# bitbank2/JPEGDEC

Hardware: NVIDIA H100
Metric: Mpixels/sec baseline 4:2:0 decode (batch) (higher is better)
Workload: dtype int16/int32 (u8 pixels)

## Files before the change

jpegdec_b200/csrc/jd_core.h:

```cpp
#ifndef JD_CORE_H
#define JD_CORE_H

#include <stdint.h>
#include <string.h>

#ifdef __CUDACC__
#define JD_HD __host__ __device__ __forceinline__
#define JD_HDM __host__ __device__ __forceinline__
#else
#define JD_HD static inline
#define JD_HDM inline
#endif

#define JD_LUT_DC_SIZE 1152
#define JD_LUT_AC_SIZE 2048
#define JD_LUT_ACF_SIZE 2048
#define JD_LUT_DC(t) ((t) * JD_LUT_DC_SIZE)
#define JD_LUT_AC(t) (2 * JD_LUT_DC_SIZE + (t) * JD_LUT_AC_SIZE)
#define JD_LUT_ACF(t) (2 * JD_LUT_DC_SIZE + 2 * JD_LUT_AC_SIZE + (t) * JD_LUT_ACF_SIZE)
#define JD_LUT_ENTRIES (2 * JD_LUT_DC_SIZE + 2 * JD_LUT_AC_SIZE + 2 * JD_LUT_ACF_SIZE)
#define JD_ACF_RARE 0x80u
#define JD_ACF_PACK(len, rs) ((uint32_t)((len) + ((rs) & 15u)) | ((uint32_t)(len) << 8) | (((uint32_t)(rs) & 15u) << 16) | \
                              ((((rs) == 0u) ? 128u : (((uint32_t)(rs) >> 4) + 1u)) << 24) | \
                              (((((rs) & 15u) >= 10u) || ((len) + ((rs) & 15u) >= 18u)) ? JD_ACF_RARE : 0u))

#define JD_REC_PER_BYTE 6u
#define JD_REC_SLOT_SLACK 128u
#define JD_REC_INDEX(byte_off, slot) (((JD_REC_PER_BYTE * (uint32_t)(byte_off)) & ~7u) + JD_REC_SLOT_SLACK * (uint32_t)(slot))
#define JD_REC_CAP(nbytes) (JD_REC_PER_BYTE * (uint32_t)(nbytes) + JD_REC_SLOT_SLACK - 8u)
#define JD_REC_BLOCK_MAX 126u

typedef unsigned long long jd_u64;

JD_HD jd_u64 jd_pack_hdr(uint32_t rec_index, int dc, uint32_t ncoef, uint32_t big, uint32_t hi, uint32_t colmask)
{
    return (jd_u64)rec_index | ((jd_u64)(uint16_t)(int16_t)dc << 32) | ((jd_u64)(ncoef & 63u) << 48) |
           ((jd_u64)(big & 1u) << 54) | ((jd_u64)(hi & 1u) << 55) | ((jd_u64)(colmask & 0xFFu) << 56);
}
#define JD_HDR_REC(h) ((uint32_t)(h))
#define JD_HDR_DC(h) ((int)(short)(uint16_t)((h) >> 32))
#define JD_HDR_NCOEF(h) ((uint32_t)((h) >> 48) & 63u)
#define JD_HDR_BIG(h) ((uint32_t)((h) >> 54) & 1u)
#define JD_HDR_HI(h) ((uint32_t)((h) >> 55) & 1u)
#define JD_HDR_COLMASK(h) ((uint32_t)((h) >> 56) & 0xFFu)

#define JD_TPOS_INIT { \
    0, 8, 1, 2, 9, 16, 24, 17, 10, 3, 4, 11, 18, 25, 32, 40, \
    33, 26, 19, 12, 5, 6, 13, 20, 27, 34, 41, 48, 56, 49, 42, 35, \
    28, 21, 14, 7, 15, 22, 29, 36, 43, 50, 57, 58, 51, 44, 37, 30, \
    23, 31, 38, 45, 52, 59, 60, 53, 46, 39, 47, 54, 61, 62, 55, 63 }
#define JD_TRANSPOSE6(x) ((((x) & 7u) << 3) | ((x) >> 3))

#define JD_DEZIGZAG_INIT { \
    0, 1, 8, 16, 9, 2, 3, 10, 17, 24, 32, 25, 18, 11, 4, 5, \
    12, 19, 26, 33, 40, 48, 41, 34, 27, 20, 13, 6, 7, 14, 21, 28, \
    35, 42, 49, 56, 57, 50, 43, 36, 29, 22, 15, 23, 30, 37, 44, 51, \
    58, 59, 52, 45, 38, 31, 39, 46, 53, 60, 61, 54, 47, 55, 62, 63 }

#define JD_JW_INIT 0x543210u
#define JD_JW_ONES 0x111111u

JD_HD uint32_t jd_jw_ckpt(uint32_t jw)
{
    uint32_t t = (jw + 0x222222u) & 0x888888u;
    uint32_t m = t | (t - (t >> 3));
    return jw & ~m;
}

typedef struct {
    uint32_t blk;
    uint32_t seg;
    uint32_t j1;
    uint16_t field;
    uint8_t s;
    uint8_t p7;
    uint32_t ord;
    uint32_t img;
} JDEvent;

JD_HD void jd_patch_record(uint16_t *rec, jd_u64 hdr, uint32_t ord, int v)
{
    const uint32_t ri = JD_HDR_REC(hdr);
    if (JD_HDR_BIG(hdr)) rec[ri + 2u * ord + 1u] = (uint16_t)(int16_t)v;
    else rec[ri + ord] = (uint16_t)((rec[ri + ord] & 0xFC00u) | ((uint32_t)v & 0x3FFu));
}

JD_HD int jd_event_value(const JDEvent *e, uint32_t jc)
{
    int lost = 8 * (int)jc + e->p7 + e->s - 64;
    uint32_t f = e->field;
    if (lost > 0) {
        if (lost >= e->s) f = 0; else f &= ~((1u << lost) - 1u);
    }
    int v = (int)f;
    if (!(e->field >> (e->s - 1))) v -= (1 << e->s) - 1;
    return v;
}

typedef struct {
    const uint8_t *data;
    uint32_t start;
    uint32_t end;
    uint32_t nmcu;
    uint32_t bpm;
    uint32_t ncomp;
    uint32_t tsel;
    uint32_t rec_index0;
    uint32_t rec_cap;
    uint32_t seg;
    uint32_t blk0;
    uint32_t al;
    uint32_t img;
    uint32_t *ring;
    uint16_t *stage;
    uint32_t skip_bits;
    uint32_t blk_first;
    uint32_t nblk;
    uint32_t midstream;
    int32_t pred[3];
} JDSegIn;
JD_HD void jd_segin_whole_interval(JDSegIn *in)
{
    in->skip_bits = 0; in->blk_first = 0; in->nblk = 0; in->midstream = 0; in->pred[0] = in->pred[1] = in->pred[2] = 0;
}

typedef struct {
    uint32_t jmap;
    int32_t err_mcu;
    uint32_t status;
    uint32_t nrec;
    uint32_t nblk_done;
#ifdef JD_ENTROPY_PROBE
    long long probe[4];
    uint32_t probe_sym;
#endif
} JDSegOut;

#if defined(JD_ENTROPY_PROBE) && defined(__CUDA_ARCH__)
#define JD_PROBE(...) __VA_ARGS__
#else
#define JD_PROBE(...)
#endif

#define JD_SEG_OK 0
#define JD_SEG_BADCODE 1
#define JD_SEG_OVERFLOW 2
#define JD_SEG_BADSIZE 3
#define JD_SEG_MISSING 4

#ifdef __CUDACC__
#define JD_LD8(p) (*(p))
#else
#define JD_LD8(p) (*(p))
#endif

JD_HD uint32_t jd_tposw(uint32_t t) { return t | (((t >> 2) & 1u) << 23) | ((1u << (t >> 3)) << 24); }
#define JD_BF_HI(bf) (((bf) >> 23) & 1u)
#define JD_BF_COLMASK(bf) ((bf) >> 24)
#define JD_BF_MASK 0xFF800000u

#define JD_MODE_BASELINE 0
#define JD_MODE_DC_SCAN 1
#define JD_MODE_PARSE_AC 2
#define JD_MODE_STORE_LOW 3
JD_HD uint32_t jd_bswap32(uint32_t w)
{
#ifdef __CUDA_ARCH__
    return __byte_perm(w, 0, 0x0123);
#else
    return __builtin_bswap32(w);
#endif
}

JD_HD int jd_extend_top(uint32_t x, uint32_t s)
{
    const uint32_t neg = ~(uint32_t)((int)x >> 31);
    const uint32_t y = x ^ neg;
#ifdef __CUDA_ARCH__
    const uint32_t mag = s ? __funnelshift_r(y, 0u, 32u - s) : 0u;
#else
    const uint32_t mag = s ? (y >> (32u - s)) : 0u;
#endif
    return (int)((mag ^ neg) - neg);
}

typedef struct { uint32_t x, y, z, w; } jd_u128;
JD_HD jd_u128 jd_ld128(const uint8_t *p)
{
    jd_u128 r;
#ifdef __CUDA_ARCH__
    const uint4 v = *reinterpret_cast<const uint4 *>(p);
    r.x = v.x; r.y = v.y; r.z = v.z; r.w = v.w;
#else
    memcpy(&r, p, 16);
#endif
    return r;
}

#ifdef __CUDA_ARCH__
struct JDTab16 {
    uint32_t base;
    __device__ __forceinline__ JDTab16(const uint16_t *p) : base((uint32_t)__cvta_generic_to_shared(p)) { asm volatile("" : "+r"(base)); }
    __device__ __forceinline__ uint32_t at(uint32_t i) const { uint16_t v; asm("ld.shared.u16 %0, [%1];" : "=h"(v) : "r"(base + 2u * i)); return v; }
};
struct JDTab32 {
    uint32_t base;
    __device__ __forceinline__ JDTab32(const uint32_t *p) : base((uint32_t)__cvta_generic_to_shared(p)) { asm volatile("" : "+r"(base)); }
    __device__ __forceinline__ uint32_t at(uint32_t i) const { uint32_t v; asm("ld.shared.u32 %0, [%1];" : "=r"(v) : "r"(base + 4u * i)); return v; }
};
#else
struct JDTab16 { const uint16_t *p; JDTab16(const uint16_t *q) : p(q) {} uint32_t at(uint32_t i) const { return p[i]; } };
struct JDTab32 { const uint32_t *p; JDTab32(const uint32_t *q) : p(q) {} uint32_t at(uint32_t i) const { return p[i]; } };
#endif

template <typename EventSink, int MODE = JD_MODE_BASELINE, bool CLEAN = false>
JD_HD void jd_decode_segment(const JDSegIn &in, const uint16_t *lut ,
                             const uint32_t *tposw ,
                             jd_u64 *blk_hdr , uint16_t *rec ,
                             EventSink &sink, JDSegOut &out)
{
    const uint32_t *words = (const uint32_t *)in.data;
    const uint32_t endw = (in.end + 3u) >> 2;
    const uint32_t wlast = in.end >> 2;
    uint32_t wi = in.start >> 2;
    uint32_t wnext = (!CLEAN && wi < endw) ? words[wi] : 0u;
    uint32_t skip = CLEAN ? 0u : (in.start & 3u);
    uint32_t ffp = 0;
    uint32_t eos = 0;
    jd_u64 bb = 0;
    int nb = 0;
    const uint8_t *const cbase = in.data + in.start;
    const uint32_t nchunk = CLEAN ? ((in.end - in.start + 15u) >> 4) : 0u;
    const jd_u128 zero128 = {0u, 0u, 0u, 0u};
    uint32_t *const ring = in.ring;
    uint32_t rd = 0, wr = 0, gi = 0;
    jd_u128 pa = zero128, pb = zero128;
    bool pend = false;
    auto ring_put = [&](uint32_t at, const jd_u128 &v) {
#ifdef __CUDA_ARCH__
        *reinterpret_cast<uint4 *>(ring + at) = make_uint4(v.x, v.y, v.z, v.w);
#else
        ring[at] = v.x; ring[at + 1] = v.y; ring[at + 2] = v.z; ring[at + 3] = v.w;
#endif
    };
    auto chunk = [&](uint32_t i) { return (i < nchunk) ? jd_ld128(cbase + 16u * i) : zero128; };
    auto topup = [&]() {
        if (pend) { ring_put(wr & 31u, pa); ring_put((wr + 4u) & 31u, pb); wr += 8u; }
        pend = (32u - (wr - rd)) >= 8u;
        if (pend) { pa = chunk(gi); pb = chunk(gi + 1u); gi += 2u; }
    };
    if (CLEAN) {
        for (uint32_t i = 0; i < 4u; i++) ring_put(4u * i, chunk(i));
        wr = 16u; gi = 4u;
        topup();
    }
    auto refill = [&]() {
#ifndef JD_REFILL_STRAIGHT
        if (CLEAN) {
            if (nb <= 32) {
                while (rd == wr) topup();
                const uint32_t w = ring[rd & 31u];
                rd++;
                bb |= (jd_u64)jd_bswap32(w) << (32 - nb);
                nb += 32;
            }
        } else
#endif
        if (CLEAN) {
            const bool need = nb <= 32;
            if (need && rd == wr) { do topup(); while (rd == wr); }
            const uint32_t w = jd_bswap32(ring[rd & 31u]);
            const uint32_t sh = need ? (uint32_t)(32 - nb) : 0u;
            const jd_u64 add = (jd_u64)w << sh;
            bb |= need ? add : 0ull;
            rd += need ? 1u : 0u;
            nb += need ? 32 : 0;
        } else
        while (nb <= 32) {
            const uint32_t w = wnext;
            wi++;
            wnext = (wi < endw) ? words[wi] : 0u;
            if ((((((~w) - 0x01010101u) & w & 0x80808080u)) | skip | ffp | eos | (uint32_t)(wi > wlast)) == 0u) {
                bb |= (jd_u64)jd_bswap32(w) << (32 - nb);
                nb += 32;
            } else if (eos) {
                nb = 64;
            } else {
                for (int i = 0; i < 4; i++) {
                    const uint32_t c = (w >> (8 * i)) & 0xFFu;
                    if (skip) { skip--; continue; }
                    if (eos) break;
                    if (wi - 1u == (in.end >> 2) && (uint32_t)i >= (in.end & 3u)) { eos = 1; break; }
                    if (ffp) {
                        ffp = 0;
                        if (c != 0u) { eos = 1; break; }
                        bb |= (jd_u64)0xFFu << (56 - nb);
                        nb += 8;
                        continue;
                    }
                    if (c == 0xFFu) { ffp = 1; continue; }
                    bb |= (jd_u64)c << (56 - nb);
                    nb += 8;
                }
                if (wi >= endw && !eos && nb <= 32) eos = 1;
            }
        }
    };

    int pred0 = in.pred[0], pred1 = in.pred[1], pred2 = in.pred[2];
    uint32_t jw = JD_JW_INIT;
    uint32_t p7 = in.skip_bits & 7u;
    if (CLEAN) {
        for (uint32_t skip = in.skip_bits; skip != 0u;) {
            refill();
            const uint32_t d = skip < 32u ? skip : 32u;
            bb <<= d; nb -= (int)d; skip -= d;
        }
    }
    uint32_t ro = 0;
#ifdef __CUDA_ARCH__
    size_t rec_g = __cvta_generic_to_global(rec);
    asm volatile("" : "+l"(rec_g));
#define JD_REC_ST(i, val) asm volatile("st.global.u16 [%0], %1;" ::"l"(rec_g + 2ull * (i)), "h"((uint16_t)(val)) : "memory")
#else
#define JD_REC_ST(i, val) (rec[(i)] = (uint16_t)(val))
#endif
    uint16_t *const stage = in.stage;
    bool direct = false;
    auto flush_chunk = [&](uint32_t first) {
#ifdef __CUDA_ARCH__
        const uint4 c = *reinterpret_cast<const uint4 *>(stage);
        asm volatile("st.global.v4.u32 [%0], {%1, %2, %3, %4};" ::"l"(rec_g + 2ull * first), "r"(c.x), "r"(c.y), "r"(c.z), "r"(c.w) : "memory");
#else
        memcpy(rec + first, stage, 16);
#endif
    };
    auto put = [&](uint32_t val) {
        if (!direct) {
            stage[ro & 7u] = (uint16_t)val;
            ro++;
            if ((ro & 7u) == 0u) flush_chunk(ro - 8u);
        } else {
            JD_REC_ST(ro, val);
            ro++;
            if ((ro & 7u) == 0u) direct = false;
        }
    };
    auto go_direct = [&]() {
        if (!direct) {
            for (uint32_t i = ro & ~7u; i < ro; i++) JD_REC_ST(i, stage[i & 7u]);
            direct = (ro & 7u) != 0u;
        }
    };
    int err = -1;
    bool last_was_eob = true;
    const JDTab16 T(lut);
    const JDTab32 T32((const uint32_t *)lut);
    const JDTab32 TP(tposw);

    const uint32_t nluma = (in.ncomp == 3) ? in.bpm - 2 : in.bpm;
    const uint32_t nblk_total = in.nblk ? in.nblk : in.nmcu * in.bpm;
    uint32_t sched = 0;
    for (uint32_t i = 0; i < in.bpm && i < 8u; i++) {
        const uint32_t c = (i < nluma) ? 0u : (i - nluma + 1u);
        sched |= (c | (((in.tsel >> (2 * c)) & 1u) << 2) | (((in.tsel >> (2 * c + 1)) & 1u) << 3)) << (4 * i);
    }
    const uint32_t bsh_end = 4u * in.bpm;
    uint32_t bsh = 4u * in.blk_first;
    constexpr uint32_t LIMIT = (MODE == JD_MODE_STORE_LOW) ? 5u : 64u;
    uint32_t b = 0;

    JD_PROBE(long long pt[4] = {0, 0, 0, 0}; long long pc0 = clock64(), pc1; uint32_t nsym = 0;)
#define JD_PROBE_MARK(s) JD_PROBE(pc1 = clock64(); pt[s] += pc1 - pc0; pc0 = pc1;)
    for (; b < nblk_total; b++) {
        const uint32_t cur = (sched >> bsh) & 15u;
        JD_PROBE_MARK(3)
        if (CLEAN) topup();
        JD_PROBE_MARK(0)
        refill();
        jw = jd_jw_ckpt(jw);
        int dcval;
        {
            const uint32_t w16 = (uint32_t)(bb >> 48);
            const uint32_t e = T.at(JD_LUT_DC((cur >> 2) & 1u) + ((w16 >= 0xF800u) ? (1024u + ((w16 >> 4) & 0x7Fu)) : (w16 >> 6)));
            if (e == 0u) { err = JD_SEG_BADCODE; break; }
            const uint32_t len = e >> 8, s = e & 15u;
            bb <<= len;
            const int v = jd_extend_top((uint32_t)(bb >> 32), s);
            bb <<= s;
            nb -= (int)(len + s);
            uint32_t t = p7 + len;
            jw += (t >> 3) * JD_JW_ONES;
            if (s != 0u && len + s > 6u) jw = jd_jw_ckpt(jw);
            t = (t & 7u) + s;
            jw += (t >> 3) * JD_JW_ONES;
            p7 = t & 7u;
            const uint32_t comp = cur & 3u;
            const int pv = ((comp == 0u) ? pred0 : ((comp == 1u) ? pred1 : pred2)) + ((MODE == JD_MODE_DC_SCAN) ? (int)((uint32_t)v << in.al) : v);
            pred0 = (comp == 0u) ? pv : pred0;
            pred1 = (comp == 1u) ? pv : pred1;
            pred2 = (comp >= 2u) ? pv : pred2;
            dcval = pv;
        }
        JD_PROBE_MARK(1)
        const uint32_t r0 = ro;
        uint32_t bflags = 0, bigm = 0;
        if (MODE != JD_MODE_DC_SCAN) {
            if (MODE != JD_MODE_PARSE_AC && in.rec_cap - ro < JD_REC_BLOCK_MAX) { err = JD_SEG_OVERFLOW; break; }
            uint32_t tacf = JD_LUT_ACF(cur >> 3) >> 1;
#if defined(__CUDA_ARCH__) && !defined(JD_NO_LAUNDER)
            asm volatile("" : "+r"(tacf));
#endif
            uint32_t k = 1;
            do {
                JD_PROBE(nsym++;)
                refill();
                jw = jd_jw_ckpt(jw);
                const uint32_t hi = (uint32_t)(bb >> 32);
                uint32_t e = T32.at(tacf + (hi >> 22));
                if (e == 0u) {
                    const uint32_t e16 = (hi >= 0xFC000000u) ? T.at(JD_LUT_AC(cur >> 3) + 1024u + ((hi >> 16) & 0x3FFu)) : 0u;
                    if (e16 == 0u) { err = JD_SEG_BADCODE; break; }
                    e = JD_ACF_PACK(e16 >> 8, e16 & 0xFFu) | JD_ACF_RARE;
                }
                const uint32_t tot = e & 0x1Fu, len = (e >> 8) & 0xFFu, s = (e >> 16) & 0xFFu;
#ifdef __CUDA_ARCH__
                const uint32_t x = __funnelshift_l((uint32_t)bb, hi, len);
                const uint32_t mag = __funnelshift_r(x, 0u, 32u - s);
#else
                const uint32_t x = (uint32_t)((bb << len) >> 32);
                const uint32_t mag = s ? (x >> (32u - s)) : 0u;
#endif
                const int v = (int)(mag - (~(uint32_t)((int)x >> 31) & ~(0xFFFFFFFFu << s)));
                bb <<= tot;
                nb -= (int)tot;
                const uint32_t kn = k + (e >> 24);
                if (MODE != JD_MODE_PARSE_AC && s != 0u && kn <= LIMIT) {
                    const uint32_t tw = TP.at(kn - 1u);
                    bflags |= tw;
                    if (((e | bigm) & JD_ACF_RARE) != 0u) {
                        if (s > 11u) { err = JD_SEG_BADSIZE; break; }
                        if (len + s >= 18u) {
                            const uint32_t t1 = p7 + len;
                            const uint32_t j1 = jw + (t1 >> 3) * JD_JW_ONES;
                            const int q7 = (int)(t1 & 7u);
                            if (((j1 + 0x222222u) & 0x888888u) != 0u) {
                                bool any = false;
                                for (int c = 0; c < 6; c++) {
                                    const int jc = (int)((j1 >> (4 * c)) & 15u);
                                    if (8 * jc + q7 + (int)s > 64) any = true;
                                }
                                if (any) {
                                    JDEvent ev;
                                    ev.blk = in.blk0 + b;
                                    ev.seg = in.seg;
                                    ev.j1 = j1;
                                    ev.field = (uint16_t)(x >> (32u - s));
                                    ev.s = (uint8_t)s;
                                    ev.p7 = (uint8_t)q7;
                                    ev.ord = bigm ? (ro - r0) >> 1 : (ro - r0);
                                    ev.img = in.img;
                                    sink.push(ev);
                                }
                            }
                        }
                        if (s >= 10u && !bigm) {
                            const uint32_t ncoef = ro - r0;
                            go_direct();
                            uint16_t *const rec0 = rec + r0;
                            for (uint32_t i = ncoef; i-- > 0u;) {
                                const uint32_t r = rec0[i];
                                rec0[2u * i] = (uint16_t)(r >> 10);
                                rec0[2u * i + 1u] = (uint16_t)(int16_t)((int)(r << 22) >> 22);
                            }
                            ro += ncoef;
                            direct = true;
                            bigm = JD_ACF_RARE;
                        }
                        if (bigm) {
                            put(tw & 63u);
                            put((uint32_t)v & 0xFFFFu);
                        } else {
                            put((tw << 10) | ((uint32_t)v & 0x3FFu));
                        }
                    } else {
                        put((tw << 10) | ((uint32_t)v & 0x3FFu));
                    }
                }
                {
                    const uint32_t t = p7 + tot;
                    jw += (t >> 3) * JD_JW_ONES;
                    p7 = t & 7u;
                }
                k = kn;
            } while (k < 64u);
            if (err >= 0) break;
            last_was_eob = (k >= 128u);
        }
        JD_PROBE_MARK(2)
        {
            const uint32_t nrec = ro - r0;
            const uint32_t cnt = (bigm ? ((nrec >> 1) << 16) | (1u << 22) : (nrec << 16));
            const uint32_t ridx0 = in.rec_index0 + r0;
            blk_hdr[b] = (jd_u64)ridx0 | ((jd_u64)((bflags & JD_BF_MASK) | cnt | ((uint32_t)dcval & 0xFFFFu)) << 32);
        }
        bsh += 4u;
        if (bsh == bsh_end) bsh = 0u;
    }
    JD_PROBE_MARK(3)
    JD_PROBE(for (int i = 0; i < 4; i++) out.probe[i] = pt[i]; out.probe_sym = nsym;)
#undef JD_PROBE_MARK
    if (!direct && (ro & 7u) != 0u) flush_chunk(ro & ~7u);
    if (err >= 0) {
        out.err_mcu = (int32_t)((b + in.blk_first) / in.bpm);
        for (uint32_t bb2 = b; bb2 < nblk_total; bb2++) blk_hdr[bb2] = jd_pack_hdr(in.rec_index0, 0, 0, 0, 0, 0);
    }
    out.status = (err < 0) ? (uint32_t)JD_SEG_OK : (uint32_t)err;
    if (err < 0) {
        out.err_mcu = -1;
        if (!in.midstream) {
            if (!last_was_eob) jw = jd_jw_ckpt(jw);
            if (p7) jw += JD_JW_ONES;
        }
    }
    out.jmap = jw;
    out.nrec = ro;
    out.nblk_done = b;
#undef JD_REC_ST
}


JD_HD uint32_t jd_range(int v)
{
    int s = (int)((uint32_t)v << 17) >> 22;
    s += 128;
    s = s < 0 ? 0 : s;
    s = s > 255 ? 255 : s;
    return (uint32_t)s;
}

JD_HD int jd_mh2(int x, int K)
{
#ifdef __CUDA_ARCH__
    return (((int)((uint32_t)x << 18) >> 16) * K) >> 16;
#else
    return (int)(((int64_t)(int32_t)((uint32_t)x << 18) * (int64_t)K) >> 32);
#endif
}

#define JD_K0414 (1697 * 4)
#define JD_K1414 (5793 * 4)
#define JD_K1847 (7568 * 4)
#define JD_K2613 (10703 * 2)
#define JD_K1082 (4433 * 4)

JD_HD void jd_col_sse16(const int d[8], bool rows47_empty, int o[8])
{
    int T0, T1, T2, T3, T4, T5, T6, T7;
    if (rows47_empty) {
        const int d0 = d[0], d1 = d[1], d2 = d[2], d3 = d[3];
        int t12 = jd_mh2(d2, JD_K0414);
        T0 = d0 + d2; T3 = d0 - d2; T1 = d0 + t12; T2 = d0 - t12;
        T7 = d1 + d3;
        int t11 = jd_mh2(d1 - d3, JD_K1414);
        int z5 = jd_mh2(d1 - d3, JD_K1847);
        t12 = 2 * jd_mh2(d3, JD_K2613) + z5;
        T6 = t12 - T7;
        T5 = t11 - T6;
        T4 = (jd_mh2(d1, JD_K1082) - z5) + T5;
    } else {
        int t10 = d[0] + d[4], t11 = d[0] - d[4];
        int t13 = d[2] + d[6];
        int t12 = jd_mh2(d[2] - d[6], JD_K1414) - t13;
        T0 = t10 + t13; T3 = t10 - t13; T1 = t11 + t12; T2 = t11 - t12;
        int z13 = d[5] + d[3], z10 = d[5] - d[3];
        int z11 = d[1] + d[7], z12 = d[1] - d[7];
        T7 = z11 + z13;
        t11 = jd_mh2(z11 - z13, JD_K1414);
        int z5 = jd_mh2(z10 + z12, JD_K1847);
        t12 = 2 * jd_mh2(z10, -JD_K2613) + z5;
        T6 = t12 - T7;
        T5 = t11 - T6;
        T4 = (jd_mh2(z12, JD_K1082) - z5) + T5;
    }
    o[0] = T0 + T7; o[1] = T1 + T6; o[2] = T2 + T5; o[3] = T3 - T4;
    o[4] = T3 + T4; o[5] = T2 - T5; o[6] = T1 - T6; o[7] = T0 - T7;
}

JD_HD void jd_col_scalar(const int m[8], const int q[8], bool rows47_empty, int o[8])
{
    int tmp0, tmp1, tmp2, tmp3, tmp4, tmp5, tmp6, tmp7, tmp10, tmp11, tmp12, tmp13, z5, z10, z11, z12, z13;
    if (rows47_empty) {
        tmp10 = m[0] * q[0];
        tmp1 = m[2] * q[2];
        tmp12 = (tmp1 * 106) >> 8;
        tmp0 = tmp10 + tmp1; tmp3 = tmp10 - tmp1; tmp1 = tmp10 + tmp12; tmp2 = tmp10 - tmp12;
        tmp4 = m[1] * q[1];
        if (m[3] != 0) {
            tmp5 = m[3] * q[3];
            tmp7 = tmp4 + tmp5;
            tmp11 = ((tmp4 - tmp5) * 362) >> 8;
            z5 = ((tmp4 - tmp5) * 473) >> 8;
            tmp12 = ((-tmp5 * -669) >> 8) + z5;
            tmp6 = tmp12 - tmp7;
            tmp5 = tmp11 - tmp6;
            tmp10 = ((tmp4 * 277) >> 8) - z5;
            tmp4 = tmp10 + tmp5;
        } else {
            tmp7 = tmp4;
            tmp5 = (145 * tmp4) >> 8;
            tmp6 = (217 * tmp4) >> 8;
            tmp4 = (-51 * tmp4) >> 8;
        }
    } else {
        tmp0 = m[0] * q[0];
        tmp2 = m[4] * q[4];
        tmp10 = tmp0 + tmp2; tmp11 = tmp0 - tmp2;
        tmp1 = m[2] * q[2];
        tmp3 = m[6] * q[6];
        tmp13 = tmp1 + tmp3;
        tmp12 = (((tmp1 - tmp3) * 362) >> 8) - tmp13;
        tmp0 = tmp10 + tmp13; tmp3 = tmp10 - tmp13; tmp1 = tmp11 + tmp12; tmp2 = tmp11 - tmp12;
        tmp5 = m[3] * q[3];
        tmp6 = m[5] * q[5];
        z13 = tmp6 + tmp5; z10 = tmp6 - tmp5;
        tmp4 = m[1] * q[1];
        tmp7 = m[7] * q[7];
        z11 = tmp4 + tmp7; z12 = tmp4 - tmp7;
        tmp7 = z11 + z13;
        tmp11 = ((z11 - z13) * 362) >> 8;
        z5 = ((z10 + z12) * 473) >> 8;
        tmp12 = ((z10 * -669) >> 8) + z5;
        tmp6 = tmp12 - tmp7;
        tmp5 = tmp11 - tmp6;
        tmp10 = ((z12 * 277) >> 8) - z5;
        tmp4 = tmp10 + tmp5;
    }
    o[0] = tmp0 + tmp7; o[1] = tmp1 + tmp6; o[2] = tmp2 + tmp5; o[3] = tmp3 - tmp4;
    o[4] = tmp3 + tmp4; o[5] = tmp2 - tmp5; o[6] = tmp1 - tmp6; o[7] = tmp0 - tmp7;
}

#define JD_MS8(x, K) (((x) * (K)) >> 8)
JD_HD void jd_row_terms(const int p[8], uint32_t colmask, int t[8])
{
    int tmp0, tmp1, tmp2, tmp3, tmp4, tmp5, tmp6, tmp7;
    if ((colmask & 0xf0u) == 0u) {
        if ((colmask & 0xfcu) == 0u) {
            tmp0 = tmp1 = tmp2 = tmp3 = p[0];
            tmp7 = p[1];
            tmp6 = JD_MS8(tmp7, 217);
            tmp5 = JD_MS8(tmp7, 145);
            tmp4 = -JD_MS8(tmp7, 51);
        } else {
            int tmp10 = p[0], tmp13 = p[2];
            int tmp12 = JD_MS8(tmp13, 106);
            tmp0 = tmp10 + tmp13; tmp3 = tmp10 - tmp13; tmp1 = tmp10 + tmp12; tmp2 = tmp10 - tmp12;
            int z13 = p[3], z11 = p[1];
            tmp7 = z11 + z13;
            int tmp11 = JD_MS8(z11 - z13, 362);
            int z5 = JD_MS8(z11 - z13, 473);
            tmp10 = JD_MS8(z11, 277) - z5;
            tmp12 = JD_MS8(z13, 669) + z5;
            tmp6 = tmp12 - tmp7;
            tmp5 = tmp11 - tmp6;
            tmp4 = tmp10 + tmp5;
// ... 233 lines not shown
```

jpegdec_b200/csrc/jd_host.c:

```c
#include <stdio.h>
#include <string.h>
#include <stdlib.h>
#include <math.h>
#include "jd_internal.h"
#include "jd_resize.h"
#include "jd_reduce.h"

#define HUFF_TABLEN 273

static unsigned be16(const uint8_t *p) { return ((unsigned)p[0] << 8) | p[1]; }

static unsigned tiff16(const uint8_t *p, int mot) { return mot ? ((unsigned)p[0] << 8) | p[1] : ((unsigned)p[1] << 8) | p[0]; }
static unsigned tiff32(const uint8_t *p, int mot)
{
    return mot ? ((unsigned)p[0] << 24) | ((unsigned)p[1] << 16) | ((unsigned)p[2] << 8) | p[3]
               : ((unsigned)p[3] << 24) | ((unsigned)p[2] << 16) | ((unsigned)p[1] << 8) | p[0];
}

static int tiff_value(const uint8_t *p, int mot)
{
    int type = (int)tiff16(p + 2, mot);
    if (tiff16(p + 4, mot) > 1) type = 4;
    switch (type) {
        case 3: return (int)tiff16(p + 8, mot);
// ... 167 lines not shown
        off += (int)len;
    }
    if (marker != 0xFFDA) return fail(info, JPEG_DECODE_ERROR);
    off -= (int)len;
    if (off + 3 > size) return fail(info, JPEG_DECODE_ERROR);
    int slen = (int)be16(s + off);
    off += 2;
    int nc = s[off++];
    info->p.ncomp_in_scan = (uint8_t)nc;
    slen -= 3;
    if (nc >= 1 && nc <= 4 && slen == nc * 2 + 3 && off + nc * 2 + 3 <= size) {
        int bad = 0;
        for (int i = 0; i < nc && !bad; i++) {
            unsigned cc = s[off++], c = s[off++];
            int j;
            for (j = 0; j < 4; j++) if (info->p.comp_id[j] == cc) break;
            if (j == 4) { bad = 1; break; }
            if ((c & 0xF) > 3 || (c & 0xF0) > 0x30) { bad = 1; break; }
            info->p.comp_dc[j] = (uint8_t)(c >> 4);
            info->p.comp_ac[j] = (uint8_t)(c & 0xF);
        }
        if (!bad) {
            info->p.scan_start = s[off++];
            info->p.scan_end = s[off++];
            info->approx = s[off++];
        }
    }
    info->scan_offset = off;
    info->p.scan_offset = off;
    if (!(prog_tables && info->mode == 0xC2) && !jd_check_huffman(info)) return fail(info, JPEG_UNSUPPORTED_FEATURE);

    if (info->ncomp != 1 && info->ncomp != 3) return fail(info, JPEG_UNSUPPORTED_FEATURE);
    switch (info->subsample) {
        case 0x00: case 0x11: info->mcu_w = 8; info->mcu_h = 8; info->bpm = (info->ncomp == 3) ? 3 : 1; break;
        case 0x21: info->mcu_w = 16; info->mcu_h = 8; info->bpm = 4; break;
        case 0x12: info->mcu_w = 8; info->mcu_h = 16; info->bpm = 4; break;
        case 0x22: info->mcu_w = 16; info->mcu_h = 16; info->bpm = 6; break;
        default: return fail(info, JPEG_UNSUPPORTED_FEATURE);
    }
    if (info->width <= 0 || info->height <= 0) return fail(info, JPEG_DECODE_ERROR);
    info->mcus_x = (info->width + info->mcu_w - 1) / info->mcu_w;
    info->mcus_y = (info->height + info->mcu_h - 1) / info->mcu_h;
    info->tsel = 0;
    info->tables_ok = 1;
    for (int c = 0; c < info->ncomp; c++) {
        if (info->p.comp_dc[c] > 1 || info->p.comp_ac[c] > 1) info->tables_ok = 0;
        info->tsel |= (info->p.comp_dc[c] & 1) << (2 * c);
        info->tsel |= (info->p.comp_ac[c] & 1) << (2 * c + 1);
    }
    info->error = JPEG_SUCCESS;
    return 1;
}

int jd_check_huffman(const JDInfo *info)
{
    const uint8_t *hv = info->p.huffvals;
    for (int t = 0; t < 4; t++) {
        if (!(info->p.huff_defined & (1u << t))) continue;
        const uint8_t *bits = hv + t * HUFF_TABLEN;
        unsigned cc = 0;
        for (int n = 1; n <= 16; n++) {
            int cnt = bits[n - 1];
            if (n > 12 && cnt > 0) return 0;
            while (cnt--) {
                int is_long = (n >= 5) && ((cc >> (n - 5)) == 0x1F);
                if (!is_long && n > 6) return 0;
                cc++;
            }
            cc <<= 1;
        }
    }
    if (info->mode == 0xC2) return 1;
    for (int t = 0; t < 4; t++) {
        if (!(info->p.huff_defined & (1u << (t + 4)))) continue;
        if (t >= 2) return 0;
        const uint8_t *bits = hv + (t + 4) * HUFF_TABLEN;
        unsigned cc = 0;
        for (int n = 1; n <= 16; n++) {
            int cnt = bits[n - 1];
            while (cnt--) {
                int is_long = (n >= 6) && ((cc >> (n - 6)) == 0x3F);
                if (!is_long && n > 10) return 0;
                cc++;
            }
            cc <<= 1;
        }
    }
    return 1;
}

void jd_build_lut(const JDInfo *info, uint16_t *lut)
{
    const uint8_t *hv = info->p.huffvals;
    memset(lut, 0, JD_LUT_ENTRIES_H * sizeof(uint16_t));
    for (int t = 0; t < 2; t++) {
        if (!(info->p.huff_defined & (1u << t))) continue;
        const uint8_t *bits = hv + t * HUFF_TABLEN, *vals = bits + 16;
        uint16_t *L = lut + t * 1152;
        unsigned cc = 0;
        for (int n = 1; n <= 16; n++) {
            int cnt = bits[n - 1];
            while (cnt--) {
                unsigned sym = *vals++;
                uint16_t e = (uint16_t)((n << 8) | (sym & 0xF));
                if (n >= 5 && n <= 12 && (cc >> (n - 5)) == 0x1F) {
                    unsigned first = (cc << (12 - n)) & 0x7F, rep = 1u << (12 - n);
                    for (unsigned i = 0; i < rep && first + i < 128; i++) L[1024 + first + i] = e;
                } else if (n <= 10) {
                    unsigned first = cc << (10 - n), rep = 1u << (10 - n);
                    for (unsigned i = 0; i < rep && first + i < 1024; i++) L[first + i] = e;
                }
                cc++;
            }
            cc <<= 1;
        }
    }
    for (int t = 0; t < 2; t++) {
        if (!(info->p.huff_defined & (1u << (t + 4)))) continue;
        const uint8_t *bits = hv + (t + 4) * HUFF_TABLEN, *vals = bits + 16;
        uint16_t *L = lut + 2 * 1152 + t * 2048;
        unsigned cc = 0;
        for (int n = 1; n <= 16; n++) {
            int cnt = bits[n - 1];
            while (cnt--) {
                unsigned sym = *vals++;
                uint16_t e = (uint16_t)((n << 8) | sym);
                if (n >= 6 && (cc >> (n - 6)) == 0x3F) {
                    unsigned first = (cc << (16 - n)) & 0x3FF, rep = 1u << (16 - n);
                    for (unsigned i = 0; i < rep && first + i < 1024; i++) L[1024 + first + i] = e;
                } else if (n <= 10) {
                    unsigned first = cc << (10 - n), rep = 1u << (10 - n);
                    for (unsigned i = 0; i < rep && first + i < 1024; i++) L[first + i] = e;
                }
                cc++;
            }
            cc <<= 1;
        }
    }
    for (int t = 0; t < 2; t++) {
        const uint16_t *L = lut + 2 * 1152 + t * 2048;
        uint16_t *F = lut + 2 * 1152 + 2 * 2048 + t * 2048;
        for (unsigned idx = 0; idx < 1024; idx++) {
            uint16_t e = 0;
            if ((idx >> 4) != 0x3F) e = L[idx];
            else {
                const uint16_t *x = L + 1024 + ((idx & 15u) << 6);
                e = x[0];
                for (int j = 1; j < 64; j++) if (x[j] != e) e = 0;
                if ((e >> 8) > 10) e = 0;
            }
            uint32_t f = 0;
            if (e) {
                const unsigned len = e >> 8, rs = e & 0xFFu, s = rs & 15u;
                f = (len + s) | (len << 8) | (s << 16) | ((rs == 0 ? 128u : (rs >> 4) + 1u) << 24);
                if (s >= 10 || len + s >= 18) f |= 0x80u;
            }
            F[2 * idx] = (uint16_t)(f & 0xFFFFu);
            F[2 * idx + 1] = (uint16_t)(f >> 16);
        }
    }
}

static const int jd_aan_scale[64] = {
    16384, 22725, 21407, 19266, 16384, 12873, 8867, 4520,
    22725, 31521, 29692, 26722, 22725, 17855, 12299, 6270,
    21407, 29692, 27969, 25172, 21407, 16819, 11585, 5906,
    19266, 26722, 25172, 22654, 19266, 15137, 10426, 5315,
    16384, 22725, 21407, 19266, 16384, 12873, 8867, 4520,
    12873, 17855, 16819, 15137, 12873, 10114, 6967, 3552,
    8867, 12299, 11585, 10426, 8867, 6967, 4799, 2446,
    4520, 6270, 5906, 5315, 4520, 3552, 2446, 1247};

const int *jd_aan_table(void) { return jd_aan_scale; }

static const uint8_t jd_zigzag_of_natural[64] = {
    0, 1, 5, 6, 14, 15, 27, 28, 2, 4, 7, 13, 16, 26, 29, 42,
    3, 8, 12, 17, 25, 30, 41, 43, 9, 11, 18, 24, 31, 40, 44, 53,
    10, 19, 23, 32, 39, 45, 52, 54, 20, 22, 33, 38, 46, 51, 55, 60,
    21, 34, 37, 47, 50, 56, 59, 61, 35, 36, 48, 49, 57, 58, 62, 63};

void jd_build_quant(const JDInfo *info, int16_t *q)
{
    for (int c = 0; c < 3; c++) {
        int t = (c < info->ncomp) ? info->p.comp_quant[c] : 0;
        const uint16_t *raw = info->p.quant_raw[t & 3];
        for (int n = 0; n < 64; n++) {
            uint16_t v;
            if (t < info->ncomp) v = (uint16_t)(((unsigned)raw[jd_zigzag_of_natural[n]] * (unsigned)jd_aan_scale[n]) >> 12);
            else v = raw[n];
            q[c * 64 + n] = (int16_t)v;
        }
    }
}

int jd_tables_equal(const JDInfo *x, const JDInfo *y)
{
    if (x->p.huff_defined != y->p.huff_defined) return 0;
    for (int t = 0; t < 8; t++) {
        if (!(x->p.huff_defined & (1u << t))) continue;
        const uint8_t *bx = x->p.huffvals + t * HUFF_TABLEN, *by = y->p.huffvals + t * HUFF_TABLEN;
        int total = 0;
        for (int i = 0; i < 16; i++) total += bx[i];
        if (total > 256) total = 256;
        if (memcmp(bx, by, (size_t)(16 + total)) != 0) return 0;
    }
    return 1;
}

uint64_t jd_tables_hash2(const JDInfo *info)
{
    uint64_t h = 0x9E3779B97F4A7C15ull;
    const uint8_t *hv = info->p.huffvals;
    for (int t = 0; t < 8; t++) {
        if (!(info->p.huff_defined & (1u << t))) continue;
        const uint8_t *b = hv + t * HUFF_TABLEN;
        int total = 0;
        for (int i = 0; i < 16; i++) total += b[i];
        if (total > 256) total = 256;
        h = (h + (uint64_t)(t + 1)) * 0xD6E8FEB86659FD93ull; h ^= h >> 32;
        for (int i = 0; i < 16 + total; i++) { h = (h + b[i]) * 0xD6E8FEB86659FD93ull; h ^= h >> 29; }
    }
    return h;
}

uint64_t jd_tables_hash(const JDInfo *info)
{
    uint64_t h = 1469598103934665603ull;
    const uint8_t *hv = info->p.huffvals;
    for (int t = 0; t < 8; t++) {
        if (!(info->p.huff_defined & (1u << t))) continue;
        const uint8_t *b = hv + t * HUFF_TABLEN;
        int total = 0;
        for (int i = 0; i < 16; i++) total += b[i];
        if (total > 256) total = 256;
        h = (h ^ (uint64_t)(t + 1)) * 1099511628211ull;
        for (int i = 0; i < 16 + total; i++) h = (h ^ b[i]) * 1099511628211ull;
    }
    return h;
}

int jd_roi_plan(int width, int height, int subsample, int restart_interval, int sshift, const int32_t *rect, JDRoiPlan *plan)
{
    const int mcu_w = (subsample == 0x21 || subsample == 0x22) ? 16 : 8;
    const int mcu_h = (subsample == 0x12 || subsample == 0x22) ? 16 : 8;
    const int out_w = (width + (1 << sshift) - 1) >> sshift, out_h = (height + (1 << sshift) - 1) >> sshift;
    const int64_t x = rect[0], y = rect[1], w = rect[2], h = rect[3];
    if (x < 0 || y < 0 || w < 1 || h < 1 || x + w > out_w || y + h > out_h) return 0;
    const int mw = mcu_w >> sshift, mh = mcu_h >> sshift;
    const int mcus_x = (width + mcu_w - 1) / mcu_w, mcus_y = (height + mcu_h - 1) / mcu_h;
    plan->mcu_x0 = (int32_t)(x / mw);
    plan->mcu_x1 = (int32_t)((x + w - 1) / mw);
    plan->mcu_y0 = (int32_t)(y / mh);
    plan->mcu_y1 = (int32_t)((y + h - 1) / mh);
    plan->mcu_end = (plan->mcu_y1 + 1) * mcus_x;
    const int total = mcus_x * mcus_y;
    const int mps = restart_interval > 0 ? restart_interval : total;
    const int nseg = (total + mps - 1) / mps;
    const int walk = (plan->mcu_end - 1) / mps + 1;
    plan->nseg_walk = walk < nseg ? walk : nseg;
    plan->out_w = (int32_t)w;
    plan->out_h = (int32_t)h;
    return 1;
}

int jd_orient_plan(int width, int height, int subsample, int restart_interval, int sshift, int k, const int32_t *rect,
                   int32_t *srect, JDRoiPlan *plan)
{
    if (k < 1 || k > 8) return 0;
    const int64_t sw = (width + (1 << sshift) - 1) >> sshift, sh = (height + (1 << sshift) - 1) >> sshift;
    const int tr = k >= 5;
    const int64_t dw = tr ? sh : sw, dh = tr ? sw : sh;
    const int64_t x = rect ? rect[0] : 0, y = rect ? rect[1] : 0, w = rect ? rect[2] : dw, h = rect ? rect[3] : dh;
    if (x < 0 || y < 0 || w < 1 || h < 1 || x + w > dw || y + h > dh) return 0;
    const int64_t ex0 = tr ? y : x, exn = tr ? h : w, ey0 = tr ? x : y, eyn = tr ? w : h;
    srect[0] = (int32_t)(((JD_ORIENT_MX >> k) & 1u) ? sw - ex0 - exn : ex0);
    srect[1] = (int32_t)(((JD_ORIENT_MY >> k) & 1u) ? sh - ey0 - eyn : ey0);
    srect[2] = (int32_t)exn;
    srect[3] = (int32_t)eyn;
    if (!jd_roi_plan(width, height, subsample, restart_interval, sshift, srect, plan)) return 0;
    plan->out_w = (int32_t)w;
    plan->out_h = (int32_t)h;
    return 1;
}

int jd_views_plan(int width, int height, int subsample, int restart_interval, int sshift, int nv, const int32_t *rois,
                  const uint8_t *ks, const int32_t *out_sizes, JDRoiPlan *plans, int32_t *srects, int32_t *ok)
{
    const int mcu_w = (subsample == 0x21 || subsample == 0x22) ? 16 : 8;
    const int mcu_h = (subsample == 0x12 || subsample == 0x22) ? 16 : 8;
    const int total = ((width + mcu_w - 1) / mcu_w) * ((height + mcu_h - 1) / mcu_h);
    const int mps = restart_interval > 0 ? restart_interval : total;
    const int nseg = (total + mps - 1) / mps;
    int walk = 0;
    for (int v = 0; v < nv; v++) {
        int32_t *sr = srects + 4 * (size_t)v;
        sr[0] = sr[1] = sr[2] = sr[3] = 0;
        int good = 1;
        if (ks) good = jd_orient_plan(width, height, subsample, restart_interval, sshift, ks[v], rois ? rois + 4 * (size_t)v : NULL,
                                      sr, &plans[v]);
        else if (rois) {
            good = jd_roi_plan(width, height, subsample, restart_interval, sshift, rois + 4 * (size_t)v, &plans[v]);
            sr[0] = rois[4 * (size_t)v]; sr[1] = rois[4 * (size_t)v + 1];
        }
        if (good && out_sizes) {
            const int32_t rw = out_sizes[2 * (size_t)v], rh = out_sizes[2 * (size_t)v + 1];
            if (rw < 1 || rw > 65535 || rh < 1 || rh > 65535) good = 0;
        }
// ... 815 lines not shown
```

Measured before the change: 245,000.

## Rebalance Huffman AC inner loop across ALU/FMA pipes and batch word loads

The fast AC lookup table now stores (32-s)&31 instead of s, so the magnitude extraction and sign mask can use funnel shifts directly on table fields without separate field extraction. The jw checkpoint and bit-position carry logic are rewritten to use __umulhi with an opaque constant, shifting work from the integer logic pipe to the multiply pipe. The non-clean bitstream reader loads 16-byte chunks into a four-word queue instead of one word per refill, and common-case puts bypass the direct-mode check via a staged variant with an end_direct fixup. Optional pipe-pressure probe macros are added, and the changes to staging and table encoding carry correctness risk.

```diff
diff --git a/jpegdec_b200/csrc/jd_core.h b/jpegdec_b200/csrc/jd_core.h
--- a/jpegdec_b200/csrc/jd_core.h
+++ b/jpegdec_b200/csrc/jd_core.h
@@ -20,7 +20,7 @@
 #define JD_LUT_ACF(t) (2 * JD_LUT_DC_SIZE + 2 * JD_LUT_AC_SIZE + (t) * JD_LUT_ACF_SIZE)
 #define JD_LUT_ENTRIES (2 * JD_LUT_DC_SIZE + 2 * JD_LUT_AC_SIZE + 2 * JD_LUT_ACF_SIZE)
 #define JD_ACF_RARE 0x80u
-#define JD_ACF_PACK(len, rs) ((uint32_t)((len) + ((rs) & 15u)) | ((uint32_t)(len) << 8) | (((uint32_t)(rs) & 15u) << 16) | \
+#define JD_ACF_PACK(len, rs) ((uint32_t)((len) + ((rs) & 15u)) | ((uint32_t)(len) << 8) | (((32u - ((uint32_t)(rs) & 15u)) & 31u) << 16) | \
                               ((((rs) == 0u) ? 128u : (((uint32_t)(rs) >> 4) + 1u)) << 24) | \
                               (((((rs) & 15u) >= 10u) || ((len) + ((rs) & 15u) >= 18u)) ? JD_ACF_RARE : 0u))
 
@@ -65,6 +65,15 @@
     uint32_t t = (jw + 0x222222u) & 0x888888u;
     uint32_t m = t | (t - (t >> 3));
     return jw & ~m;
+}
+
+JD_HD uint32_t jd_mulhi(uint32_t a, uint32_t b)
+{
+#ifdef __CUDA_ARCH__
+    return __umulhi(a, b);
+#else
+    return (uint32_t)(((uint64_t)a * b) >> 32);
+#endif
 }
 
 typedef struct {
@@ -142,6 +151,28 @@
 #define JD_PROBE(...)
 #endif
 
+#if defined(__CUDA_ARCH__) && (defined(JD_PIPE_PROBE_ALU) || defined(JD_PIPE_PROBE_FMA))
+#define JD_PIPE_PROBE_DECL(q) \
+    uint32_t q[4] = {in.seg, in.seg ^ 0x9E3779B9u, in.start, in.start ^ 0x7F4A7C15u}; \
+    uint32_t q##_a = in.nmcu | 1u, q##_b = in.bpm ^ 0x5bd1e995u; \
+    asm volatile("" : "+r"(q##_a), "+r"(q##_b));
+#define JD_PIPE_PROBE_SINK(q) { *reinterpret_cast<uint32_t *>(in.stage) = q[0] + q[1] + q[2] + q[3]; }
+#ifdef JD_PIPE_PROBE_ALU
+#define JD_PIPE_PROBE_INJECT(q) \
+    _Pragma("unroll") for (int pi_ = 0; pi_ < JD_PIPE_PROBE_ALU; pi_++) { \
+        if ((pi_ >> 2) & 1) asm volatile("lop3.b32 %0, %0, %1, %2, 0x96;" : "+r"(q[pi_ & 3]) : "r"(q##_a), "r"(q##_b)); \
+        else asm volatile("shf.l.wrap.b32 %0, %0, %1, %2;" : "+r"(q[pi_ & 3]) : "r"(q##_b), "r"(q##_a)); }
+#else
+#define JD_PIPE_PROBE_INJECT(q) \
+    _Pragma("unroll") for (int pi_ = 0; pi_ < JD_PIPE_PROBE_FMA; pi_++) \
+        asm volatile("mad.lo.u32 %0, %0, %1, %2;" : "+r"(q[pi_ & 3]) : "r"(q##_a), "r"(q##_b));
+#endif
+#else
+#define JD_PIPE_PROBE_DECL(q)
+#define JD_PIPE_PROBE_SINK(q)
+#define JD_PIPE_PROBE_INJECT(q)
+#endif
+
 #define JD_SEG_OK 0
 #define JD_SEG_BADCODE 1
 #define JD_SEG_OVERFLOW 2
@@ -223,7 +254,23 @@
     const uint32_t endw = (in.end + 3u) >> 2;
     const uint32_t wlast = in.end >> 2;
     uint32_t wi = in.start >> 2;
-    uint32_t wnext = (!CLEAN && wi < endw) ? words[wi] : 0u;
+    uint32_t q0 = 0u, q1 = 0u, q2 = 0u, q3 = 0u, qn = 0u;
+    auto qload = [&](uint32_t c) {
+        if (c + 4u <= endw) {
+            const jd_u128 v = jd_ld128((const uint8_t *)(words + c));
+            q0 = v.x; q1 = v.y; q2 = v.z; q3 = v.w;
+        } else {
+            q0 = (c < endw) ? words[c] : 0u;
+            q1 = (c + 1u < endw) ? words[c + 1u] : 0u;
+            q2 = (c + 2u < endw) ? words[c + 2u] : 0u;
+            q3 = 0u;
+        }
+    };
+    if (!CLEAN) {
+        qload(wi & ~3u);
+        for (uint32_t i = wi & ~3u; i < wi; i++) { q0 = q1; q1 = q2; q2 = q3; }
+        qn = 4u - (wi & 3u);
+    }
     uint32_t skip = CLEAN ? 0u : (in.start & 3u);
     uint32_t ffp = 0;
     uint32_t eos = 0;
@@ -277,9 +324,10 @@
             nb += need ? 32 : 0;
         } else
         while (nb <= 32) {
-            const uint32_t w = wnext;
+            const uint32_t w = q0;
             wi++;
-            wnext = (wi < endw) ? words[wi] : 0u;
+            q0 = q1; q1 = q2; q2 = q3;
+            if (--qn == 0u) { qload(wi); qn = 4u; }
             if ((((((~w) - 0x01010101u) & w & 0x80808080u)) | skip | ffp | eos | (uint32_t)(wi > wlast)) == 0u) {
                 bb |= (jd_u64)jd_bswap32(w) << (32 - nb);
                 nb += 32;
@@ -352,6 +400,17 @@
             direct = (ro & 7u) != 0u;
         }
     };
+    auto end_direct = [&]() {
+        if (direct) {
+            for (uint32_t i = ro & ~7u; i < ro; i++) stage[i & 7u] = rec[i];
+            direct = false;
+        }
+    };
+    auto put_staged = [&](uint32_t val) {
+        stage[ro & 7u] = (uint16_t)val;
+        ro++;
+        if ((ro & 7u) == 0u) flush_chunk(ro - 8u);
+    };
     int err = -1;
     bool last_was_eob = true;
     const JDTab16 T(lut);
@@ -370,6 +429,11 @@
     constexpr uint32_t LIMIT = (MODE == JD_MODE_STORE_LOW) ? 5u : 64u;
     uint32_t b = 0;
 
+    uint32_t k29 = 1u << 29;
+#ifdef __CUDA_ARCH__
+    asm volatile("" : "+r"(k29));
+#endif
+    JD_PIPE_PROBE_DECL(pq)
     JD_PROBE(long long pt[4] = {0, 0, 0, 0}; long long pc0 = clock64(), pc1; uint32_t nsym = 0;)
 #define JD_PROBE_MARK(s) JD_PROBE(pc1 = clock64(); pt[s] += pc1 - pc0; pc0 = pc1;)
     for (; b < nblk_total; b++) {
@@ -414,8 +478,12 @@
             uint32_t k = 1;
             do {
                 JD_PROBE(nsym++;)
+                JD_PIPE_PROBE_INJECT(pq)
                 refill();
-                jw = jd_jw_ckpt(jw);
+                {
+                    const uint32_t t8 = (jw + 0x222222u) & 0x888888u;
+                    jw &= ~jd_mulhi(t8 * 15u, k29);
+                }
                 const uint32_t hi = (uint32_t)(bb >> 32);
                 uint32_t e = T32.at(tacf + (hi >> 22));
                 if (e == 0u) {
@@ -423,22 +491,26 @@
                     if (e16 == 0u) { err = JD_SEG_BADCODE; break; }
                     e = JD_ACF_PACK(e16 >> 8, e16 & 0xFFu) | JD_ACF_RARE;
                 }
-                const uint32_t tot = e & 0x1Fu, len = (e >> 8) & 0xFFu, s = (e >> 16) & 0xFFu;
-#ifdef __CUDA_ARCH__
-                const uint32_t x = __funnelshift_l((uint32_t)bb, hi, len);
-                const uint32_t mag = __funnelshift_r(x, 0u, 32u - s);
-#else
-                const uint32_t x = (uint32_t)((bb << len) >> 32);
-                const uint32_t mag = s ? (x >> (32u - s)) : 0u;
-#endif
-                const int v = (int)(mag - (~(uint32_t)((int)x >> 31) & ~(0xFFFFFFFFu << s)));
+                const uint32_t tot = e & 0x1Fu;
+#ifdef __CUDA_ARCH__
+                const uint32_t x = __funnelshift_l((uint32_t)bb, hi, e >> 8);
+                const uint32_t mag = __funnelshift_r(x, 0u, e >> 16);
+                const uint32_t mask = __funnelshift_r(0xFFFFFFFFu, 0u, e >> 16);
+#else
+                const uint32_t s0 = (32u - ((e >> 16) & 31u)) & 31u;
+                const uint32_t x = (uint32_t)((bb << ((e >> 8) & 31u)) >> 32);
+                const uint32_t mag = s0 ? (x >> (32u - s0)) : 0u;
+                const uint32_t mask = s0 ? (0xFFFFFFFFu >> (32u - s0)) : 0u;
+#endif
+                const int v = (int)(mag - (~(uint32_t)((int)x >> 31) & mask));
                 bb <<= tot;
                 nb -= (int)tot;
                 const uint32_t kn = k + (e >> 24);
-                if (MODE != JD_MODE_PARSE_AC && s != 0u && kn <= LIMIT) {
+                if (MODE != JD_MODE_PARSE_AC && (e & 0x1F0000u) != 0u && kn <= LIMIT) {
                     const uint32_t tw = TP.at(kn - 1u);
                     bflags |= tw;
                     if (((e | bigm) & JD_ACF_RARE) != 0u) {
+                        const uint32_t len = (e >> 8) & 31u, s = tot - len;
                         if (s > 11u) { err = JD_SEG_BADSIZE; break; }
                         if (len + s >= 18u) {
                             const uint32_t t1 = p7 + len;
@@ -484,17 +556,19 @@
                             put((tw << 10) | ((uint32_t)v & 0x3FFu));
                         }
                     } else {
-                        put((tw << 10) | ((uint32_t)v & 0x3FFu));
+                        put_staged((tw << 10) | ((uint32_t)v & 0x3FFu));
                     }
                 }
                 {
                     const uint32_t t = p7 + tot;
-                    jw += (t >> 3) * JD_JW_ONES;
-                    p7 = t & 7u;
+                    const uint32_t c = jd_mulhi(t, k29);
+                    jw += c * JD_JW_ONES;
+                    p7 = t - 8u * c;
                 }
                 k = kn;
             } while (k < 64u);
             if (err >= 0) break;
+            if (bigm) end_direct();
             last_was_eob = (k >= 128u);
         }
         JD_PROBE_MARK(2)
@@ -511,6 +585,7 @@
     JD_PROBE(for (int i = 0; i < 4; i++) out.probe[i] = pt[i]; out.probe_sym = nsym;)
 #undef JD_PROBE_MARK
     if (!direct && (ro & 7u) != 0u) flush_chunk(ro & ~7u);
+    JD_PIPE_PROBE_SINK(pq)
     if (err >= 0) {
         out.err_mcu = (int32_t)((b + in.blk_first) / in.bpm);
         for (uint32_t bb2 = b; bb2 < nblk_total; bb2++) blk_hdr[bb2] = jd_pack_hdr(in.rec_index0, 0, 0, 0, 0, 0);
diff --git a/jpegdec_b200/csrc/jd_host.c b/jpegdec_b200/csrc/jd_host.c
--- a/jpegdec_b200/csrc/jd_host.c
+++ b/jpegdec_b200/csrc/jd_host.c
@@ -343,7 +343,7 @@
             uint32_t f = 0;
             if (e) {
                 const unsigned len = e >> 8, rs = e & 0xFFu, s = rs & 15u;
-                f = (len + s) | (len << 8) | (s << 16) | ((rs == 0 ? 128u : (rs >> 4) + 1u) << 24);
+                f = (len + s) | (len << 8) | (((32u - s) & 31u) << 16) | ((rs == 0 ? 128u : (rs >> 4) + 1u) << 24);
                 if (s >= 10 || len + s >= 18) f |= 0x80u;
             }
             F[2 * idx] = (uint16_t)(f & 0xFFFFu);
```

After: 245,300, median of 6. No clear change (+0.1%).
